# tum-vision/povar

Hardware: AMD Instinct MI355X
Metric: power-series iterations/s (solve_pOSE terms per second) (higher is better)
Workload: dtype f64

## Files before the change

povar_amd/csrc/ck_layout.hpp:

```cpp
#pragma once

#include <climits>
#include <cmath>
#include <cstring>

#include "lpl_layout.hpp"

namespace povar {

#ifndef POVAR_CK_HMAX_BUILD
#define POVAR_CK_HMAX_BUILD 16
#endif
constexpr int CK_HMAX = POVAR_CK_HMAX_BUILD;
constexpr int CK_LDS_BYTES = 160 * 1024;
constexpr int CK_FLAG_DUP = 1;
constexpr int CK_FLAG_COLD = 2;
constexpr uint32_t CK_NONE = 0xffffu;

constexpr double CK_UV_SCALE = 1e6, CK_UV_INV = 1e-6;
inline double ck_unpack_uv_host(int32_t k) {
  const double kd = (double)k;
  const double q0 = kd * CK_UV_INV;
  const double r = std::fma(-q0, CK_UV_SCALE, kd);
  return std::fma(r, CK_UV_INV, q0);
// ... 164 lines not shown
  std::vector<int> lcnt(L.tile.size() * WAVE, 0);
  lpl_parallel(grid, n_threads, [&](int w) {
    WgOut& o = out[w];
    o.bt_tiles.assign(nb, 0);
    const int t0 = L.wg_tile_off[w], t1 = L.wg_tile_off[w + 1];
    struct Ob { int key, li, src; };
    const int n_par_w = L.wg_cam_off[w + 1] - L.wg_cam_off[w];
    const int n_acc_w = std::min(n_par_w, max_acc);
    std::vector<int> acc_of_slot(n_par_w);
    std::vector<int>& acc_rank = acc_rank_of[w];
    acc_rank.resize(n_acc_w);
    if (n_acc_w == n_par_w) {
      for (int sl = 0; sl < n_par_w; ++sl) { acc_of_slot[sl] = sl; acc_rank[sl] = L.wg_cams[L.wg_cam_off[w] + sl]; }
    } else {
      std::vector<long> cnt(n_par_w, 0);
      for (int t = L.wg_tile_off[w]; t < L.wg_tile_off[w + 1]; ++t) {
        const int4 ti = L.tile[t];
        for (size_t idx = (size_t)ti.x * WAVE; idx < ((size_t)ti.x + ti.y) * WAVE; ++idx)
          if (L.cw[idx] >= 0) cnt[lpl_cw_slot(L.cw[idx])]++;
      }
      std::vector<int> by_cnt(n_par_w);
      for (int sl = 0; sl < n_par_w; ++sl) by_cnt[sl] = sl;
      std::stable_sort(by_cnt.begin(), by_cnt.end(), [&](int a, int c) { return cnt[a] > cnt[c]; });
      std::vector<char> keep(n_par_w, 0);
      for (int i = 0; i < n_acc_w; ++i) keep[by_cnt[i]] = 1;
      int a = 0;
      for (int sl = 0; sl < n_par_w; ++sl) {
        acc_of_slot[sl] = keep[sl] ? a : -1;
        if (keep[sl]) acc_rank[a++] = L.wg_cams[L.wg_cam_off[w] + sl];
        else o.capped += cnt[sl];
      }
    }
    std::vector<Ob> obs;
    std::vector<int> counts, first_of;
    struct Chunk { int key, first, len; };
    std::vector<Chunk> chunks;
    std::vector<int> assign;
    std::vector<long> cost;
    for (int b = 0; b < nb; ++b) {
      obs.clear();
      for (int t = t0 + b; t < t1; t += nb) {
        const int4 ti = L.tile[t];
        const int slot0 = ((t - t0) / nb) * WAVE;
        for (int j = 0; j < ti.y; ++j)
          for (int lane = 0; lane < WAVE; ++lane) {
            const size_t idx = ((size_t)ti.x + j) * WAVE + lane;
            const int cw = L.cw[idx];
            if (cw == -1) continue;
            Ob ob;
            if (cw >= 0) {
              const int sl = lpl_cw_slot(cw), a = acc_of_slot[sl];
              ob.key = a >= 0 ? a : n_acc_w + L.wg_cams[L.wg_cam_off[w] + sl];
            } else {
              ob.key = n_acc_w + (-2 - cw);
            }
            ob.li = slot0 + (L.seg[(size_t)t * WAVE + lane] & 255);
            ob.src = (int)idx;
            obs.push_back(ob);
            lcnt[(size_t)t * WAVE + (L.seg[(size_t)t * WAVE + lane] & 255)]++;
          }
      }
      o.obs += (int64_t)obs.size();
      std::stable_sort(obs.begin(), obs.end(), [](const Ob& a, const Ob& c) { return a.key < c.key; });
      counts.clear();
      first_of.clear();
      for (size_t i = 0; i < obs.size();) {
        size_t j = i;
        while (j < obs.size() && obs[j].key == obs[i].key) ++j;
        counts.push_back((int)(j - i));
        first_of.push_back((int)i);
        i = j;
      }
      int H = hmax, best = INT_MAX;
      for (int h = std::min(2, hmax); h <= hmax; ++h) {
        const int c = ck_schedule_cost(counts, h, n_waves, tile_overhead, nullptr);
        if (c <= best) { best = c; H = h; }
      }
      chunks.clear();
      for (size_t g = 0; g < counts.size(); ++g) {
        const int n = counts[g], k = (n + H - 1) / H, base = n / k, rem = n % k;
        int at = first_of[g];
        for (int q = 0; q < k; ++q) {
          const int len = base + (q < rem ? 1 : 0);
          chunks.push_back(Chunk{obs[at].key, at, len});
          at += len;
        }
      }
      auto rank_of = [&](int key) { return key >= n_acc_w ? key - n_acc_w : acc_rank[key]; };
      std::stable_sort(chunks.begin(), chunks.end(), [&](const Chunk& a, const Chunk& c) {
        if (a.len != c.len) return a.len > c.len;
        const int ra = rank_of(a.key), rc = rank_of(c.key);
        return ra != rc ? ra < rc : a.key < c.key;
      });
      o.chunks += (int64_t)chunks.size();
      const int n_tiles = ((int)chunks.size() + WAVE - 1) / WAVE;
      o.bt_tiles[b] = n_tiles;
      for (int tt = 0; tt < n_tiles; ++tt) {
        const int c0 = tt * WAVE, c1 = std::min((int)chunks.size(), c0 + WAVE);
        const int T = chunks[c0].len;
        int4 ti = make_int4((int)(o.uv.size() / WAVE), T, 0, (int)(o.li.size() / WAVE));
        const size_t r0 = o.uv.size(), q0 = o.li.size();
        o.uv.resize(r0 + (size_t)T * WAVE, make_double2(0, 0));
        if (shape.cold_q) o.cpos.resize(r0 + (size_t)T * WAVE, -1);
        o.src.resize(r0 + (size_t)T * WAVE, -1);
        o.li.resize(q0 + (size_t)((T + 1) / 2) * WAVE, CK_NONE | (CK_NONE << 16));
        const size_t l0 = o.lane_cam.size();
        o.lane_cam.resize(l0 + WAVE, -1);
        o.lane_acc.resize(l0 + WAVE, 0);
        o.lane_seg.resize(l0 + WAVE, 0);
        for (int lane = 0; lane < WAVE; ++lane) o.lane_seg[l0 + lane] = lane | (lane << 8);
        uint16_t occ[CK_HMAX][2][32] = {};
        uint16_t mx[CK_HMAX][2];
        for (int j = 0; j < CK_HMAX; ++j) mx[j][0] = mx[j][1] = 1;
        for (int q = c0; q < c1; ++q) {
          const int lane = q - c0, half = lane >> 5;
          const Chunk& ck = chunks[q];
          const bool cold = ck.key >= n_acc_w;
          o.lane_cam[l0 + lane] = cold ? ck.key - n_acc_w : acc_rank[ck.key];
          if (cold) {
            if (shape.cold_q) {
              o.lane_acc[l0 + lane] = -1;
              ++o.n_cold_q;
            } else {
              o.lane_acc[l0 + lane] = ~(int)o.cold_rank.size();
              o.cold_rank.push_back(ck.key - n_acc_w);
            }
            ti.z |= CK_FLAG_COLD;
          } else {
            o.lane_acc[l0 + lane] = ck.key;
            if (lane > 0 && chunks[q - 1].key == ck.key) ti.z |= CK_FLAG_DUP;
          }
          const int h = ck.len;
          assign.resize(h);
          if (place && T > 1) {
            cost.assign((size_t)T * T, 0);
            for (int a = 0; a < h; ++a) {
              const int cls = obs[ck.first + a].li & 31;
              for (int j = 0; j < T; ++j) {
                const int v = occ[j][half][cls];
                cost[(size_t)a * T + j] = 1000L * std::max(0, v + 1 - (int)mx[j][half]) + v;
              }
            }
            std::vector<int> full;
            lpl_assign(T, cost, full);
            for (int a = 0; a < h; ++a) assign[a] = full[a];
          } else {
            for (int a = 0; a < h; ++a) assign[a] = a;
          }
          for (int a = 0; a < h; ++a) {
            const Ob& ob = obs[ck.first + a];
            const int j = assign[a];
            const size_t idx = r0 + (size_t)j * WAVE + lane;
            const size_t s = (size_t)ob.src;
            o.uv[idx] = L.uv[s];
            if (shape.cold_q && cold) o.cpos[idx] = L.cpos[s];
            o.src[idx] = ob.src;
            uint32_t& word = o.li[q0 + (size_t)(j >> 1) * WAVE + lane];
            const uint32_t li3 = (uint32_t)shape.li_mul * (uint32_t)ob.li;
            word = (j & 1) ? ((word & 0xffffu) | (li3 << 16)) : ((word & 0xffff0000u) | li3);
            const uint16_t v = ++occ[j][half][ob.li & 31];
            mx[j][half] = std::max(mx[j][half], v);
          }
        }
        for (int j = 0; j < T; ++j) o.extra += (mx[j][0] - 1) + (mx[j][1] - 1);
        if (ti.z & CK_FLAG_DUP) {
          int lane = 0;
          const int nl = c1 - c0;
          while (lane < nl) {
            int e = lane;
            if (o.lane_acc[l0 + lane] >= 0)
              while (e + 1 < nl && o.lane_acc[l0 + e + 1] == o.lane_acc[l0 + lane]) ++e;
            for (int x = lane; x <= e; ++x) o.lane_seg[l0 + x] = lane | (e << 8);
            lane = e + 1;
          }
        }
        o.tile.push_back(ti);
      }
    }
  });
  K.bt_off.assign((size_t)grid * nb + 1, 0);
  std::vector<int64_t> row0_of(grid), li0_of(grid);
  std::vector<int> tile0_of(grid), cold0_of(grid);
  int n_cold_chunks = 0;
  int64_t n_cold_q = 0;
  for (int w = 0; w < grid; ++w) {
    const WgOut& o = out[w];
    row0_of[w] = K.rows;
    li0_of[w] = K.li_rows;
    tile0_of[w] = (int)K.tile.size();
    cold0_of[w] = n_cold_chunks;
    n_cold_chunks += (int)o.cold_rank.size();
    n_cold_q += o.n_cold_q;
    int t = (int)K.tile.size();
    for (int b = 0; b < nb; ++b) {
      K.bt_off[(size_t)w * nb + b] = t;
      t += o.bt_tiles[b];
      K.max_tiles_bt = std::max(K.max_tiles_bt, o.bt_tiles[b]);
    }
    for (int4 ti : o.tile) {
      ti.x += (int)K.rows;
      ti.w += (int)K.li_rows;
      K.tile.push_back(ti);
    }
    K.rows += (int64_t)(o.uv.size() / WAVE);
    K.li_rows += (int64_t)(o.li.size() / WAVE);
    K.n_chunks += o.chunks;
    K.n_obs += o.obs;
    K.n_capped_obs += o.capped;
    K.extra_lanes += o.extra;
  }
  K.bt_off[(size_t)grid * nb] = (int)K.tile.size();
  K.n_cold_chunks = n_cold_chunks + n_cold_q;
  K.cold_q = shape.cold_q;
  auto clog2 = [](int n) { int e = 0; while ((1 << e) < n) ++e; return (uint8_t)(n == 0 ? 255 : e); };
  K.lcnt_log2.resize(lcnt.size());
  for (size_t i = 0; i < lcnt.size(); ++i) K.lcnt_log2[i] = clog2(lcnt[i]);

  std::vector<int> n_rec(n_cams, 0);
  for (int w = 0; w < grid; ++w)
    for (int r0 : acc_rank_of[w]) n_rec[r0]++;
  std::vector<int> n_slot_rec(n_rec);
  for (int w = 0; w < grid; ++w)
    for (int r0 : out[w].cold_rank) n_rec[r0]++;
  std::vector<int> first(n_cams + 1, 0);
  for (int r0 = 0; r0 < n_cams; ++r0) first[r0 + 1] = first[r0] + n_rec[r0];
  K.n_part_rec = first[n_cams];
  K.part_range.assign(n_cams, make_int2(0, 0));
  for (int r0 = 0; r0 < n_cams; ++r0) K.part_range[cam_of_rank[r0]] = make_int2(first[r0], first[r0 + 1]);
  K.slot_rec.assign(L.wg_cams.size(), 0);
  {
    std::vector<int> next(first.begin(), first.end() - 1);
    for (int w = 0; w < grid; ++w)
      for (size_t a = 0; a < acc_rank_of[w].size(); ++a) K.slot_rec[(size_t)L.wg_cam_off[w] + a] = next[acc_rank_of[w][a]]++;
    std::vector<int> cold_rec((size_t)n_cold_chunks);
    for (int w = 0; w < grid; ++w)
      for (size_t i = 0; i < out[w].cold_rank.size(); ++i) cold_rec[(size_t)cold0_of[w] + i] = next[out[w].cold_rank[i]]++;
    K.uv.assign((size_t)(K.rows + CK_HMAX) * WAVE, make_double2(0, 0));
    K.src.assign((size_t)(K.rows + CK_HMAX) * WAVE, -1);
    if (shape.cold_q) K.cpos.assign((size_t)(K.rows + CK_HMAX) * WAVE, -1);
    K.li.assign((size_t)(K.li_rows + CK_HMAX) * WAVE, CK_NONE | (CK_NONE << 16));
    K.lane_cam.resize(K.tile.size() * WAVE);
    K.lane_acc.resize(K.tile.size() * WAVE);
    K.lane_seg.resize(K.tile.size() * WAVE);
    lpl_parallel(grid, n_threads, [&](int w) {
      const WgOut& o = out[w];
      std::copy(o.uv.begin(), o.uv.end(), K.uv.begin() + row0_of[w] * WAVE);
      std::copy(o.src.begin(), o.src.end(), K.src.begin() + row0_of[w] * WAVE);
      if (shape.cold_q) std::copy(o.cpos.begin(), o.cpos.end(), K.cpos.begin() + row0_of[w] * WAVE);
      std::copy(o.li.begin(), o.li.end(), K.li.begin() + li0_of[w] * WAVE);
      std::copy(o.lane_cam.begin(), o.lane_cam.end(), K.lane_cam.begin() + (size_t)tile0_of[w] * WAVE);
      std::copy(o.lane_seg.begin(), o.lane_seg.end(), K.lane_seg.begin() + (size_t)tile0_of[w] * WAVE);
      for (size_t i = 0; i < o.lane_acc.size(); ++i) {
        const int a = o.lane_acc[i];
        K.lane_acc[(size_t)tile0_of[w] * WAVE + i] = a >= 0 ? a : shape.cold_q ? -1 : ~cold_rec[(size_t)cold0_of[w] + (size_t)(~a)];
      }
    });
  }
  K.n_uv = K.uv.size();
  {
    const char* e = std::getenv("POVAR_CK_PACK");
    if (shape.need_uv && shape.slot_bytes == 48 && pack_uv && !(e && e[0] == '0')) ck_pack_uv(K, n_threads);
  }
  K.tick.assign(K.tile.size() * WAVE, 0);
  lpl_parallel(grid, n_threads, [&](int w) {
    std::vector<int> next((size_t)std::max(1, L.wg_cam_off[w + 1] - L.wg_cam_off[w]), 0);
    for (int b = 0; b < nb; ++b) {
      const int tb0 = K.bt_off[(size_t)w * nb + b], tb1 = K.bt_off[(size_t)w * nb + b + 1];
      for (int q0 = tb0; q0 < tb1; q0 += n_waves)
        for (int t = std::min(q0 + n_waves, tb1) - 1; t >= q0; --t)
          for (int lane = 0; lane < WAVE; ++lane) {
            const size_t i = (size_t)t * WAVE + lane;
            if (K.lane_cam[i] >= 0 && K.lane_acc[i] >= 0 && lane == ((K.lane_seg[i] >> 8) & 255))
              K.tick[i] = (uint16_t)next[K.lane_acc[i]]++;
          }
    }
  });
}

constexpr int CK_FIRST_PLANES = 4;
inline int ck_first_gw(int plane) { return plane == 0 ? 16 : plane == 1 ? 12 : 8; }
inline int ck_first_ng(int plane) { return plane == 3 ? 2 : 1; }
inline void ck_first_tables(const CkLayout& K, int grid, std::vector<int2>& meta, std::vector<int4>& hdr) {
  meta.assign((size_t)CK_FIRST_PLANES * grid * 16 * WAVE, make_int2(0xffff | (0xffff << 16), -1));
  hdr.assign((size_t)CK_FIRST_PLANES * grid * 16, make_int4(0, 0, 0, 0));
  const int nb = K.nb;
  auto rank16 = [&](int t, int lane) { const int r = K.lane_cam[(size_t)t * WAVE + lane]; return r < 0 ? 0xffff : (r & 0xffff); };
  for (int p = 0; p < CK_FIRST_PLANES; ++p) {
    const int gw = ck_first_gw(p), ng = ck_first_ng(p);
    for (int w = 0; w < grid; ++w)
      for (int s = 0; s < ng * gw; ++s) {
        const int b = s / gw, j = s % gw;
        if (b >= nb) continue;
        const int tb0 = K.bt_off[(size_t)w * nb + b], tb1 = K.bt_off[(size_t)w * nb + b + 1];
        const int t = tb0 + j, t2 = tb0 + gw + (gw - 1 - j);
        if (t >= tb1) continue;
        const size_t at = ((size_t)p * grid + w) * 16 + s;
        hdr[at] = K.tile[t];
        for (int lane = 0; lane < WAVE; ++lane)
          meta[at * WAVE + lane] = make_int2(rank16(t, lane) | ((t2 < tb1 ? rank16(t2, lane) : 0xffff) << 16), t);
      }
  }
}

}
```

povar_amd/csrc/povar_kernels_ck.hpp:

```cpp
#pragma once

#include "povar_kernels.hpp"

namespace povar {

constexpr int CK_ROWS = 16;

struct CkP {
  const double2* uv;
  const uint32_t* li;
  const double* w;
  const int4* tile;
  const int2* lane_meta;
  const int* bt_off;
  const int* slot_rec;
  int nb, slots;
  unsigned uv_bytes, li_bytes;
  const uint8_t* lcnt;
  const uint16_t* tick;
  int max_acc;
  int uv_packed;
  const int* cpos;
  double4* q4c;
  const int2* first_meta;
  const int4* first_hdr;
};
__device__ inline double ck_unpack_uv(unsigned k) {
  const double kd = (double)(int)k;
  const double q0 = kd * 1e-6;
  const double r = __builtin_fma(-q0, 1e6, kd);
  return __builtin_fma(r, 1e-6, q0);
}
typedef unsigned __attribute__((ext_vector_type(4))) ck_u4;
constexpr int CK_ACC_STRIDE = 13;
__host__ __device__ inline size_t ck_lds_bytes_dev(int slots, int n_acc, int ng) { return 16 + (size_t)ng * slots * 48 + (size_t)n_acc * CK_ACC_STRIDE * 8 + 64; }

__device__ inline void ck_barrier() { asm volatile("s_waitcnt lgkmcnt(0)\n\ts_barrier" ::: "memory"); }

__device__ inline void ck_group_barrier(int* cnt, int& gen, int group_waves, int lane) {
  asm volatile("s_waitcnt lgkmcnt(0)" ::: "memory");
  gen += group_waves;
  if (lane == 0) __hip_atomic_fetch_add(cnt, 1, __ATOMIC_RELAXED, __HIP_MEMORY_SCOPE_WORKGROUP);
  while (__hip_atomic_load(cnt, __ATOMIC_RELAXED, __HIP_MEMORY_SCOPE_WORKGROUP) < gen) __builtin_amdgcn_s_sleep(2);
  asm volatile("" ::: "memory");
}

__host__ __device__ inline int ck_rank(int x) { return x < 0 ? -1 : (x & 0xffff); }
__host__ __device__ inline int ck_seg(int x) { return ((x >> 16) & 63) | (((x >> 22) & 63) << 8); }

__device__ inline void ck_forward_math(const LplObs& o, const double* zz, const double* P3, double hx, double hy, double hz,
                                       double* red) {
  const double d0 = hx * zz[0] + hy * zz[1] + hz * zz[2] + zz[3];
  const double d1 = hx * zz[4] + hy * zz[5] + hz * zz[6] + zz[7];
  const double d2 = hx * zz[8] + hy * zz[9] + hz * zz[10] + zz[11];
  const double a0 = o.w * (d0 - o.cu * d2);
  const double a1 = o.w * (d1 - o.cv * d2);
  const double a2 = o.w * (o.cuv * d2 - o.cu * d0 - o.cv * d1);
  red[0] = P3[0] * a0 + P3[3] * a1 + P3[6] * a2;
  red[1] = P3[1] * a0 + P3[4] * a1 + P3[7] * a2;
  red[2] = P3[2] * a0 + P3[5] * a1 + P3[8] * a2;
}

__device__ inline double ck_huber_w(const Dp& d, const double* P3, double hx, double hy, double hz, double2 uv) {
  const double p0 = P3[0] * hx + P3[1] * hy + P3[2] * hz + P3[9];
  const double p1 = P3[3] * hx + P3[4] * hy + P3[5] * hz + P3[10];
  const double p2 = P3[6] * hx + P3[7] * hy + P3[8] * hz + P3[11];
  const double a = p0 - uv.x * p2, b = p1 - uv.y * p2, c = p0 - uv.x, e = p1 - uv.y;
  const double r2 = d.sb * d.sb * (a * a + b * b) + d.sa * d.sa * (c * c + e * e);
  const double t = d.huber;
  double y = __builtin_amdgcn_rsq(r2);
  const double hr = 0.5 * r2;
  y = y * __builtin_fma(-hr * y, y, 1.5);
  y = y * __builtin_fma(-hr * y, y, 1.5);
  return r2 < t * t ? 1.0 : t * y;
}

__device__ inline void ck_obs_forward(const Dp& d, double2 uv, double w, const double* zz, const double* P3, double hx, double hy,
                                      double hz, double* lu, int S, uint32_t s) {
  LplObs o;
  o.set(d, uv, w);
  double red[3];
  ck_forward_math(o, zz, P3, hx, hy, hz, red);
  __hip_atomic_fetch_add(lu + s, red[0], __ATOMIC_RELAXED, __HIP_MEMORY_SCOPE_WORKGROUP);
  __hip_atomic_fetch_add(lu + s + 1, red[1], __ATOMIC_RELAXED, __HIP_MEMORY_SCOPE_WORKGROUP);
  __hip_atomic_fetch_add(lu + s + 2, red[2], __ATOMIC_RELAXED, __HIP_MEMORY_SCOPE_WORKGROUP);
}
__device__ inline void ck_obs_backward(const Dp& d, double2 uv, double w, const double* P3, double hx, double hy, double hz,
                                       const double* g, double* y) {
  LplObs o;
  o.set(d, uv, w);
  double q[3];
  lpl_backward(o, P3, g, q);
#pragma unroll
  for (int m = 0; m < 3; ++m) {
    y[4 * m] += hx * q[m];
    y[4 * m + 1] += hy * q[m];
    y[4 * m + 2] += hz * q[m];
    y[4 * m + 3] += q[m];
  }
}

struct CkRows {
  __amdgpu_buffer_rsrc_t uv, li, w;
};
__device__ inline CkRows ck_rows(const CkP& k) {
  CkRows R;
  R.uv = __builtin_amdgcn_make_buffer_rsrc(const_cast<double2*>(k.uv), 0, k.uv_bytes, 0x00020000);
  R.li = __builtin_amdgcn_make_buffer_rsrc(const_cast<uint32_t*>(k.li), 0, k.li_bytes, 0x00020000);
  R.w = __builtin_amdgcn_make_buffer_rsrc(const_cast<double*>(k.w), 0, k.w ? (k.uv_packed ? k.uv_bytes : k.uv_bytes / 2) : 0, 0x00020000);
  return R;
}
template <int D, bool ROBUST, bool PK = false>
struct CkStream {
  double2 uv[D];
  unsigned pk[D][2];
  uint32_t w[D];
  __device__ inline void clear() {
#pragma unroll
    for (int i = 0; i < D; ++i) {
      uv[i] = make_double2(0, 0);
      pk[i][0] = pk[i][1] = 0;
      w[i] = 0xffffffffu;
    }
  }
  __device__ inline double2 get(int i) const { return PK ? make_double2(ck_unpack_uv(pk[i][0]), ck_unpack_uv(pk[i][1])) : uv[i]; }
  __device__ inline void load(const CkRows& R, int row0, int li0, int j, int h, int lane, int i) {
    j = j < 0 ? 0 : (j >= h ? h - 1 : j);
    const unsigned ul = (unsigned)lane;
    const unsigned ro = (unsigned)(row0 + j) * (unsigned)(WAVE * 16), lo = (unsigned)(li0 + (j >> 1)) * (unsigned)(WAVE * 4);
    if (PK) {
      typedef unsigned __attribute__((ext_vector_type(2))) u2;
      const u2 a = __builtin_amdgcn_raw_buffer_load_b64(R.uv, ul * 8u, ro >> 1, 0);
      pk[i][0] = a.x;
      pk[i][1] = a.y;
    } else {
      typedef unsigned __attribute__((ext_vector_type(4))) u4;
      const u4 a = __builtin_amdgcn_raw_buffer_load_b128(R.uv, ul * 16u, ro, 0);
      uv[i] = make_double2(__longlong_as_double(((long long)a.y << 32) | a.x), __longlong_as_double(((long long)a.w << 32) | a.z));
    }
    w[i] = __builtin_amdgcn_raw_buffer_load_b32(R.li, ul * 4u, lo, 0);
  }
  template <int DIR>
  __device__ inline void start(const CkRows& R, int row0, int li0, int h, int lane) {
#pragma unroll
    for (int i = 0; i < D; ++i) load(R, row0, li0, DIR > 0 ? i : h - 1 - i, h, lane, i);
  }
};
template <int D, bool ROBUST, bool PK>
__device__ inline void ck_forward_step(const Dp& d, const CkRows& k, CkStream<D, ROBUST, PK>& st, int row0, int li0, int h, int lane,
                                       const double* zz, const double* P3, const double* lh, double* lu, int S, int j, int i) {
  const double2 uv = st.get(i);
  const uint32_t s = (st.w[i] >> (16 * (j & 1))) & 0xffffu;
  st.load(k, row0, li0, j + D, h, lane, i);
  if (s != 0xffffu) {
    const double hx = lh[s], hy = lh[s + 1], hz = lh[s + 2];
    const double rw = ROBUST ? ck_huber_w(d, P3, hx, hy, hz, uv) : 1.0;
    ck_obs_forward(d, uv, rw, zz, P3, hx, hy, hz, lu, S, s);
  }
}
template <int D, bool ROBUST, bool PK>
__device__ inline void ck_forward_rows(const Dp& d, const CkRows& k, CkStream<D, ROBUST, PK>& st, int row0, int li0, int h, int lane,
                                       const double* zz, const double* P3, const double* lh, double* lu, int S) {
  int n0 = 0;
#pragma nounroll
  for (; n0 + D <= h; n0 += D) {
#pragma unroll
    for (int i = 0; i < D; ++i) ck_forward_step<D, ROBUST, PK>(d, k, st, row0, li0, h, lane, zz, P3, lh, lu, S, n0 + i, i);
  }
#pragma unroll
  for (int i = 0; i < D - 1; ++i)
    if (n0 + i < h) ck_forward_step<D, ROBUST, PK>(d, k, st, row0, li0, h, lane, zz, P3, lh, lu, S, n0 + i, i);
}
template <int D, bool ROBUST, bool PK>
__device__ inline void ck_backward_step(const Dp& d, const CkRows& k, CkStream<D, ROBUST, PK>& st, int row0, int li0, int h, int lane,
                                        const double* P3, const double* lh, const double* lg, int S, double* y, int j, int i) {
  const double2 uv = st.get(i);
  const uint32_t s = (st.w[i] >> (16 * (j & 1))) & 0xffffu;
  st.load(k, row0, li0, j - D, h, lane, i);
  if (s != 0xffffu) {
    const double hx = lh[s], hy = lh[s + 1], hz = lh[s + 2];
    const double rw = ROBUST ? ck_huber_w(d, P3, hx, hy, hz, uv) : 1.0;
    const double g[3] = {lg[s], lg[s + 1], lg[s + 2]};
    ck_obs_backward(d, uv, rw, P3, hx, hy, hz, g, y);
  }
}
template <int D, bool ROBUST, bool PK>
__device__ inline void ck_backward_rows(const Dp& d, const CkRows& k, CkStream<D, ROBUST, PK>& st, int row0, int li0, int h, int lane,
                                        const double* P3, const double* lh, const double* lg, int S, double* y) {
  int n0 = 0;
#pragma nounroll
  for (; n0 + D <= h; n0 += D) {
#pragma unroll
    for (int i = 0; i < D; ++i) ck_backward_step<D, ROBUST, PK>(d, k, st, row0, li0, h, lane, P3, lh, lg, S, y, h - 1 - (n0 + i), i);
  }
#pragma unroll
  for (int i = 0; i < D - 1; ++i)
    if (n0 + i < h) ck_backward_step<D, ROBUST, PK>(d, k, st, row0, li0, h, lane, P3, lh, lg, S, y, h - 1 - (n0 + i), i);
}

template <bool ROBUST, bool PK>
__device__ inline void ck_backward_rows_cold(const Dp& d, const CkP& k, const CkRows& R, int row0, int li0, int h, int lane,
                                             const double* P3, const double* lh, const double* lg, bool cold_lane, double* y) {
  for (int j = h - 1; j >= 0; --j) {
    CkStream<2, ROBUST, PK> one;
    one.load(R, row0, li0, j, h, lane, 0);
    const int cp = cold_lane ? k.cpos[(size_t)(row0 + j) * WAVE + lane] : -1;
    const double2 uv = one.get(0);
    const uint32_t s = (one.w[0] >> (16 * (j & 1))) & 0xffffu;
    if (s != 0xffffu) {
      const double hx = lh[s], hy = lh[s + 1], hz = lh[s + 2];
      const double rw = ROBUST ? ck_huber_w(d, P3, hx, hy, hz, uv) : 1.0;
      const double g[3] = {lg[s], lg[s + 1], lg[s + 2]};
      LplObs o;
      o.set(d, uv, rw);
      double q[3];
      lpl_backward(o, P3, g, q);
      if (cp >= 0) {
        k.q4c[cp] = make_double4(q[0], q[1], q[2], 0.0);
      } else {
#pragma unroll
        for (int m = 0; m < 3; ++m) {
          y[4 * m] += hx * q[m];
          y[4 * m + 1] += hy * q[m];
          y[4 * m + 2] += hz * q[m];
          y[4 * m + 3] += q[m];
        }
      }
    }
  }
}

__device__ inline void ck_load_z(const Dp& d, int rank, double* zz) {
  const double2* r = reinterpret_cast<const double2*>(d.hot_rec + (size_t)rank * HOT_REC_STRIDE);
#pragma unroll
  for (int j = 0; j < 6; ++j) {
    const double2 v = r[j];
    zz[2 * j] = v.x;
    zz[2 * j + 1] = v.y;
  }
}
__device__ inline __amdgpu_buffer_rsrc_t ck_zimg_rsrc(const Dp& d) {
  return __builtin_amdgcn_make_buffer_rsrc(d.zimg, 0, (unsigned)d.n_cams * 96u, 0x00020000);
}
__device__ inline void ck_load_z_img(const Dp& d, int rank, double* zz) {
  const __amdgpu_buffer_rsrc_t ZR = ck_zimg_rsrc(d);
#pragma unroll
  for (int j = 0; j < 6; ++j) {
    const ck_u4 a = __builtin_amdgcn_raw_buffer_load_b128(ZR, (unsigned)rank * 96u + 16u * j, 0, 0);
    zz[2 * j] = __hiloint2double((int)a.y, (int)a.x);
    zz[2 * j + 1] = __hiloint2double((int)a.w, (int)a.z);
  }
}
__device__ inline void ck_load_p3(const Dp& d, int rank, double* P3) {
  const double2* r = reinterpret_cast<const double2*>(d.hot_rec + (size_t)rank * HOT_REC_STRIDE) + 6;
#pragma unroll
  for (int j = 0; j < 4; ++j) {
    const double2 v = r[j];
    P3[2 * j] = v.x;
    P3[2 * j + 1] = v.y;
  }
  P3[8] = d.hot_rec[(size_t)rank * HOT_REC_STRIDE + 20];
}
template <bool ROBUST>
__device__ inline void ck_load_p(const Dp& d, int rank, double* P3) {
  ck_load_p3(d, rank, P3);
  if (ROBUST) {
    const double* r = d.hot_rec + (size_t)rank * HOT_REC_STRIDE;
    P3[9] = r[21];
    const double2 v = reinterpret_cast<const double2*>(r)[11];
    P3[10] = v.x;
    P3[11] = v.y;
  }
}

#ifndef POVAR_CK_PART_AUX
#define POVAR_CK_PART_AUX 0
#endif
__device__ inline __amdgpu_buffer_rsrc_t ck_part_rsrc(double* part_out) {
  return __builtin_amdgcn_make_buffer_rsrc(part_out, 0, 0x7ffffff0, 0x00020000);
}
__device__ inline void ck_store_part(__amdgpu_buffer_rsrc_t pr, unsigned byte_off, double a, double b) {
  ck_u4 g;
  g.x = (unsigned)__double2loint(a); g.y = (unsigned)__double2hiint(a); g.z = (unsigned)__double2loint(b); g.w = (unsigned)__double2hiint(b);
  __builtin_amdgcn_raw_buffer_store_b128(g, pr, byte_off, 0, POVAR_CK_PART_AUX);
}
__device__ inline void ck_flush_tile(double (&y)[12], int flags, int lane, int rank, int acc_slot, int seg, double* acc, int n_acc,
                                     double* part_ptr) {
  if (flags & 1) seg_scan_steps<12>(y, lane, seg & 255, 4);
  if (rank >= 0) {
    if (acc_slot >= 0) {
      if (lane == ((seg >> 8) & 255)) {
#pragma unroll
        for (int m = 0; m < 12; ++m)
          __hip_atomic_fetch_add(acc + acc_slot * CK_ACC_STRIDE + m, y[m], __ATOMIC_RELAXED, __HIP_MEMORY_SCOPE_WORKGROUP);
      }
    } else if (part_ptr) {
      const __amdgpu_buffer_rsrc_t part_out = ck_part_rsrc(part_ptr);
      const unsigned o = (unsigned)(~acc_slot) * 96u;
#pragma unroll
      for (int m = 0; m < 6; ++m) ck_store_part(part_out, o + 16u * m, y[2 * m], y[2 * m + 1]);
    }
  }
}

template <int NW, int SD, bool DB, int NG, bool ROBUST, bool PK>
__global__ __launch_bounds__(NW * 64) void e0_ck(Dp d, CkP k, double* part_out) {
  const int done = d.flags[1];
  extern __shared__ double ck_lds[];
  constexpr int GW = NW / NG;
  const CkRows R = ck_rows(k);
  const int S = k.slots;
  const int lane0 = threadIdx.x & 63;
  const int wave_all = __builtin_amdgcn_readfirstlane((int)(threadIdx.x >> 6));
  const int grp = NG > 1 ? wave_all / GW : 0;
  const int wave = NG > 1 ? wave_all % GW : wave_all;
  int* gbase = reinterpret_cast<int*>(ck_lds);
  double* lh = ck_lds + 2 + (size_t)grp * 6 * S;
  double* lu = lh + 3 * S;
  double* acc = ck_lds + 2 + (size_t)NG * 6 * S;
  int* gcnt = gbase + grp;
  int ggen = 0;
  const V2& v = d.v2;
  const int cam0 = v.wg_cam_off[blockIdx.x];
  const int n_acc = v.wg_cam_off[blockIdx.x + 1] - cam0;
  const int t0 = __builtin_amdgcn_readfirstlane(v.wg_tile_off[blockIdx.x]);
  const int t1 = __builtin_amdgcn_readfirstlane(v.wg_tile_off[blockIdx.x + 1]);
  typedef const int __attribute__((address_space(4))) * cint_p;
  const cint_p tiles = (cint_p)(uintptr_t)k.tile;
  const cint_p bt = (cint_p)(uintptr_t)k.bt_off;
  if (done) return;
  auto group_barrier = [&]() {
    if (NG > 1) ck_group_barrier(gcnt, ggen, GW, lane0);
    else ck_barrier();
  };
  const int wave_t = (wave & ~3) | (((wave >> 2) & 1) ? 3 - (wave & 3) : (wave & 3));
  auto tile_of = [&](int tb0, int q) { return tb0 + q * GW + ((q & 1) ? GW - 1 - wave_t : wave_t); };
  constexpr int HM = 32 / NW > 0 ? 32 / NW : 1;
  double hn[HM][3];
  auto request_h = [&](int b, int lane) {
#pragma unroll
    for (int q = 0; q < HM; ++q) {
      hn[q][0] = hn[q][1] = hn[q][2] = 0;
      const int m = wave + q * GW;
      if (b < k.nb && t0 + b + k.nb * m < t1) {
        const double* rp = v.lmrec + ((size_t)(t0 + b + k.nb * m) * 9) * WAVE + lane;
        hn[q][0] = rp[0]; hn[q][1] = rp[WAVE]; hn[q][2] = rp[2 * WAVE];
      }
    }
  };
  int* lbt = reinterpret_cast<int*>(acc + (size_t)k.max_acc * CK_ACC_STRIDE);
  const bool bt_lds = k.nb + 1 <= 16;
  auto bt_of = [&](int i, bool first) {
    return (bt_lds && !first) ? __builtin_amdgcn_readfirstlane(lbt[i]) : bt[blockIdx.x * k.nb + i];
  };
  constexpr bool EARLY = !ROBUST && SD == 2;
  int tb0_next = 0, tb1_next = 0, rank_next = 0, rank_next2 = 0;
  ck_u4 hdr_next = {0, 0, 0, 0};
  auto request_first_meta = [&](int b, int lane, bool ranks) {
    tb0_next = tb1_next = 0;
    if (b < k.nb) {
      tb0_next = bt_of(b, b == grp);
      tb1_next = bt_of(b + 1, b == grp);
    }
    if (!ranks) return;
    rank_next = rank_next2 = 0;
    hdr_next = ck_u4{0, 0, 0, 0};
    if (b < k.nb) {
      const int tf = tile_of(tb0_next, 0), tf2 = tile_of(tb0_next, 1);
      if (tf < tb1_next && !EARLY) rank_next = ck_rank(k.lane_meta[(size_t)tf * WAVE + lane].x);
      if (tf < tb1_next && EARLY) {
        const __amdgpu_buffer_rsrc_t TR = __builtin_amdgcn_make_buffer_rsrc(const_cast<int4*>(k.tile), 0, 0x7ffffff0, 0x00020000);
        hdr_next = __builtin_amdgcn_raw_buffer_load_b128(TR, 0u, (unsigned)tf * 16u, 0);
        rank_next = ck_rank(k.lane_meta[(size_t)tf * WAVE + lane].x);
        if (tf2 < tb1_next) rank_next2 = ck_rank(k.lane_meta[(size_t)tf2 * WAVE + lane].x);
      }
    }
  };
  double zz[12] = {0, 0, 0, 0, 0, 0, 0, 0, 0, 0, 0, 0}, P3[12] = {0, 0, 0, 0, 0, 0, 0, 0, 0, 0, 0, 0};
  CkStream<SD, ROBUST, PK> st;
  st.clear();
  int row0 = 0, h = 0, fl = 0, li0 = 0;
  auto request_first_tile = [&](int lane, bool have) {
    const int tf = tile_of(tb0_next, 0);
    const int rk = rank_next < 0 ? 0 : rank_next;
    if (have && EARLY) {
      row0 = __builtin_amdgcn_readfirstlane((int)hdr_next.x);
      h = __builtin_amdgcn_readfirstlane((int)hdr_next.y);
      fl = __builtin_amdgcn_readfirstlane((int)hdr_next.z);
      li0 = __builtin_amdgcn_readfirstlane((int)hdr_next.w);
      ck_load_z_img(d, rk, zz);
      ck_load_p<ROBUST>(d, rk, P3);
      st.template start<1>(R, row0, li0, h, lane);
    } else if (have) {
      const int tf2 = tile_of(tb0_next, 1);
      row0 = tiles[4 * tf]; h = tiles[4 * tf + 1]; fl = tiles[4 * tf + 2]; li0 = tiles[4 * tf + 3];
      if (tf2 < tb1_next) rank_next2 = ck_rank(k.lane_meta[(size_t)tf2 * WAVE + lane].x);
      ck_load_p<ROBUST>(d, rk, P3);
      st.template start<1>(R, row0, li0, h, lane);
      ck_load_z_img(d, rk, zz);
    } else {
#pragma unroll
      for (int e = 0; e < 12; ++e) zz[e] = P3[e] = 0;
      st.clear();
      row0 = h = fl = li0 = 0;
    }
  };
  int bt_first = 0;
  if (bt_lds && (int)threadIdx.x <= k.nb) bt_first = k.bt_off[blockIdx.x * k.nb + threadIdx.x];
  if (EARLY) {
    static_assert(!EARLY || (NG == 1 && (GW == 16 || GW == 12 || GW == 8)) || (NG == 2 && GW == 8), "shape without a first-request table");
    constexpr int PLANE = NG > 1 ? 3 : GW == 16 ? 0 : GW == 12 ? 1 : 2;
    const unsigned fs = (PLANE * gridDim.x + blockIdx.x) * 16u + (unsigned)(grp * GW + wave_t);
    const int2 fm = k.first_meta[(size_t)fs * WAVE + lane0];
    const __amdgpu_buffer_rsrc_t HR = __builtin_amdgcn_make_buffer_rsrc(const_cast<int4*>(k.first_hdr), 0, 0x7ffffff0, 0x00020000);
    hdr_next = __builtin_amdgcn_raw_buffer_load_b128(HR, 0u, fs * 16u, 0);
    request_h(grp, lane0);
    const int r1 = fm.x & 0xffff, r2 = (fm.x >> 16) & 0xffff;
    rank_next = r1 == 0xffff ? -1 : r1;
    rank_next2 = r2 == 0xffff ? -1 : r2;
    request_first_tile(lane0, __builtin_amdgcn_readfirstlane(fm.y) >= 0);
    request_first_meta(grp, lane0, false);
  } else {
    request_first_meta(grp, lane0, true);
    request_h(grp, lane0);
  }
  for (int i = threadIdx.x; i < n_acc * CK_ACC_STRIDE; i += NW * 64) acc[i] = 0;
  if (NG > 1 && threadIdx.x < NG) gbase[threadIdx.x] = 0;
  if (bt_lds && (int)threadIdx.x <= k.nb) lbt[threadIdx.x] = bt_first;
  if (NG > 1) ck_barrier();
  for (int b = grp; b < k.nb; b += NG) {
    int lane = lane0;
    asm volatile("" : "+v"(lane));
    const int tb0 = tb0_next, tb1 = tb1_next;
    int q_t = 0;
    int t = tile_of(tb0, 0);
    int rank = rank_next;
    int tn = tile_of(tb0, 1);
    if (!EARLY) request_first_tile(lane, t < tb1);
    int rank_n = rank_next2, rank_nn = 0;
    double zn[12] = {0, 0, 0, 0, 0, 0, 0, 0, 0, 0, 0, 0}, Pn[12] = {0, 0, 0, 0, 0, 0, 0, 0, 0, 0, 0, 0};
    CkStream<SD, ROBUST, PK> stn;
    stn.clear();
    int row0n = 0, hnx = 0, fln = 0, li0n = 0;
#pragma unroll
    for (int q = 0; q < HM; ++q) {
      const int m = wave + q * GW;
      if (t0 + b + k.nb * m < t1) {
        const int s = m * WAVE + lane;
        lh[3 * s] = hn[q][0];
        lh[3 * s + 1] = hn[q][1];
        lh[3 * s + 2] = hn[q][2];
        lu[3 * s] = 0;
        lu[3 * s + 1] = 0;
        lu[3 * s + 2] = 0;
      }
    }
    for (int m = wave + HM * GW; t0 + b + k.nb * m < t1; m += GW) {
      const double* rp = v.lmrec + ((size_t)(t0 + b + k.nb * m) * 9) * WAVE + lane;
      const int s = m * WAVE + lane;
      lh[3 * s] = rp[0];
      lh[3 * s + 1] = rp[WAVE];
      lh[3 * s + 2] = rp[2 * WAVE];
      lu[3 * s] = 0;
      lu[3 * s + 1] = 0;
      lu[3 * s + 2] = 0;
    }
    auto request_next_fwd = [&]() {
      if (DB && tn < tb1) {
        const int tnn = tile_of(tb0, q_t + 2);
        row0n = tiles[4 * tn]; hnx = tiles[4 * tn + 1]; fln = tiles[4 * tn + 2]; li0n = tiles[4 * tn + 3];
        if (tnn < tb1) rank_nn = ck_rank(k.lane_meta[(size_t)tnn * WAVE + lane].x);
        const int rk = rank_n < 0 ? 0 : rank_n;
        ck_load_z_img(d, rk, zn);
        ck_load_p<ROBUST>(d, rk, Pn);
        stn.template start<1>(R, row0n, li0n, hnx, lane);
      }
    };
    request_next_fwd();
    group_barrier();
#pragma unroll
    for (int e = 0; e < 12; ++e) asm volatile("" : "+v"(zz[e]));
    while (t < tb1) {
      ck_forward_rows<SD, ROBUST, PK>(d, R, st, row0, li0, h, lane, zz, P3, lh, lu, S);
      if (tn >= tb1) break;
      t = tn;
      ++q_t;
      rank = rank_n;
      tn = tile_of(tb0, q_t + 1);
      if (DB) {
#pragma unroll
        for (int e = 0; e < 12; ++e) zz[e] = zn[e];
#pragma unroll
        for (int e = 0; e < (ROBUST ? 12 : 9); ++e) P3[e] = Pn[e];
        st = stn;
        row0 = row0n; h = hnx; fl = fln; li0 = li0n;
        rank_n = rank_nn;
        request_next_fwd();
      } else {
        row0 = tiles[4 * t]; h = tiles[4 * t + 1]; fl = tiles[4 * t + 2]; li0 = tiles[4 * t + 3];
        if (tn < tb1) rank_n = ck_rank(k.lane_meta[(size_t)tn * WAVE + lane].x);
        const int rk = rank < 0 ? 0 : rank;
        ck_load_z_img(d, rk, zz);
        ck_load_p<ROBUST>(d, rk, P3);
        st.template start<1>(R, row0, li0, h, lane);
      }
    }
    asm volatile("" : "+v"(lane));
    int acc_slot = 0, seg = 0;
    int tp = q_t > 0 ? tile_of(tb0, q_t - 1) : tb1;
    int rank_p = 0, acc_p = 0, seg_p = 0, rank_pp = 0, acc_pp = 0, seg_pp = 0;
    double G[HM][6];
#pragma unroll
    for (int q = 0; q < HM; ++q) {
#pragma unroll
      for (int e = 0; e < 6; ++e) G[q][e] = 0;
      const int m = wave + q * GW;
      if (t0 + b + k.nb * m < t1) {
        const double* rp = v.lmrec + ((size_t)(t0 + b + k.nb * m) * 9 + 3) * WAVE + lane;
#pragma unroll
        for (int e = 0; e < 6; ++e) G[q][e] = rp[e * WAVE];
      }
    }
    if (t < tb1) {
      const int2 me = k.lane_meta[(size_t)t * WAVE + lane];
      seg = ck_seg(me.x);
      acc_slot = me.y;
      if (tp < tb1) {
        const int2 mp = k.lane_meta[(size_t)tp * WAVE + lane];
        rank_p = ck_rank(mp.x);
        seg_p = ck_seg(mp.x);
        acc_p = mp.y;
      }
      st.template start<-1>(R, row0, li0, h, lane);
    }
    group_barrier();
    request_first_meta(b + NG, lane, true);
    request_h(b + NG, lane);
#pragma unroll
    for (int q = 0; q < HM; ++q) {
      const int m = wave + q * GW;
      if (t0 + b + k.nb * m < t1) {
        const int s = m * WAVE + lane;
        const double u0 = lu[3 * s], u1 = lu[3 * s + 1], u2 = lu[3 * s + 2];
        lu[3 * s] = G[q][0] * u0 + G[q][1] * u1 + G[q][2] * u2;
        lu[3 * s + 1] = G[q][1] * u0 + G[q][3] * u1 + G[q][4] * u2;
        lu[3 * s + 2] = G[q][2] * u0 + G[q][4] * u1 + G[q][5] * u2;
      }
    }
    for (int m = wave + HM * GW; t0 + b + k.nb * m < t1; m += GW) {
      const double* rp = v.lmrec + ((size_t)(t0 + b + k.nb * m) * 9 + 3) * WAVE + lane;
      const double g0 = rp[0], g1 = rp[WAVE], g2 = rp[2 * WAVE], g3 = rp[3 * WAVE], g4 = rp[4 * WAVE], g5 = rp[5 * WAVE];
      const int s = m * WAVE + lane;
      const double u0 = lu[3 * s], u1 = lu[3 * s + 1], u2 = lu[3 * s + 2];
      lu[3 * s] = g0 * u0 + g1 * u1 + g2 * u2;
      lu[3 * s + 1] = g1 * u0 + g3 * u1 + g4 * u2;
      lu[3 * s + 2] = g2 * u0 + g4 * u1 + g5 * u2;
    }
    auto request_next_bwd = [&]() {
      if (DB && tp < tb1) {
        const int tpp = q_t > 1 ? tile_of(tb0, q_t - 2) : tb1;
        row0n = tiles[4 * tp]; hnx = tiles[4 * tp + 1]; fln = tiles[4 * tp + 2]; li0n = tiles[4 * tp + 3];
        if (tpp < tb1) {
          const int2 mp = k.lane_meta[(size_t)tpp * WAVE + lane];
          rank_pp = ck_rank(mp.x);
          seg_pp = ck_seg(mp.x);
          acc_pp = mp.y;
        }
        ck_load_p<ROBUST>(d, rank_p < 0 ? 0 : rank_p, Pn);
        stn.template start<-1>(R, row0n, li0n, hnx, lane);
      }
    };
    request_next_bwd();
    group_barrier();
    while (t < tb1) {
      double y[12];
#pragma unroll
      for (int m = 0; m < 12; ++m) y[m] = 0;
      const bool cold_q = !ROBUST && k.cpos != nullptr && (fl & 2) != 0;
      if (cold_q) ck_backward_rows_cold<ROBUST, PK>(d, k, R, row0, li0, h, lane, P3, lh, lu, rank >= 0 && acc_slot < 0, y);
      else ck_backward_rows<SD, ROBUST, PK>(d, R, st, row0, li0, h, lane, P3, lh, lu, S, y);
      ck_flush_tile(y, fl, lane, rank, acc_slot, seg, acc, n_acc, cold_q ? nullptr : part_out);
      if (tp >= tb1) break;
      t = tp;
      --q_t;
      rank = rank_p; acc_slot = acc_p; seg = seg_p;
      tp = q_t > 0 ? tile_of(tb0, q_t - 1) : tb1;
      if (DB) {
#pragma unroll
        for (int e = 0; e < (ROBUST ? 12 : 9); ++e) P3[e] = Pn[e];
        st = stn;
        row0 = row0n; h = hnx; fl = fln; li0 = li0n;
        rank_p = rank_pp; acc_p = acc_pp; seg_p = seg_pp;
        request_next_bwd();
      } else {
        row0 = tiles[4 * t]; h = tiles[4 * t + 1]; fl = tiles[4 * t + 2]; li0 = tiles[4 * t + 3];
        if (tp < tb1) {
          const int2 mp = k.lane_meta[(size_t)tp * WAVE + lane];
          rank_p = ck_rank(mp.x);
          seg_p = ck_seg(mp.x);
          acc_p = mp.y;
        }
        ck_load_p<ROBUST>(d, rank < 0 ? 0 : rank, P3);
        st.template start<-1>(R, row0, li0, h, lane);
      }
    }
    if (EARLY) request_first_tile(lane, tile_of(tb0_next, 0) < tb1_next);
    group_barrier();
  }
  if (NG > 1) ck_barrier();
  const __amdgpu_buffer_rsrc_t PR = ck_part_rsrc(part_out);
  for (int i = threadIdx.x; i < n_acc * 6; i += NW * 64) {
    const int r = i / 6, m = 2 * (i % 6);
    const int rec = k.slot_rec[cam0 + r];
    ck_store_part(PR, (unsigned)rec * 96u + 16u * (unsigned)(i % 6), acc[r * CK_ACC_STRIDE + m], acc[r * CK_ACC_STRIDE + m + 1]);
  }
  if (d.p2p_epoch && blockIdx.x == 0 && threadIdx.x == 0) *d.p2p_epoch += 1;
}

POVAR_KERNEL __launch_bounds__(256) void ck_gather_w(const int* src, const double* w_lpl, double* w_ck, int64_t n) {
  const int64_t i = (int64_t)blockIdx.x * 256 + threadIdx.x;
  if (i >= n) return;
  const int s = src[i];
  w_ck[i] = s >= 0 ? w_lpl[s] : 0.0;
}

}
```

Baseline: 19390.

## Defer lane-meta decoding and add optional ticket-based barrier scheduling

For the early, single-group, 16-wave shape, the per-block lane-meta decode is deferred: raw metadata is loaded before the barrier and decoded after it, and the next-block meta and h prefetch is moved after the G·u update so it overlaps differently. A ticket mechanism is added, built on an atomic counter in LDS. It can redistribute the G-matrix loads across the first-arriving waves and let late waves use a hardware barrier instead of spinning. The ticket paths are disabled by default (POVAR_CK_TICKET=0), but the deferral path is always on for matching shapes. This changes register live ranges and barrier timing in exchange for hiding metadata load latency.

```diff
diff --git a/povar_amd/csrc/ck_layout.hpp b/povar_amd/csrc/ck_layout.hpp
--- a/povar_amd/csrc/ck_layout.hpp
+++ b/povar_amd/csrc/ck_layout.hpp
@@ -490,4 +490,10 @@
   }
 }
 
-}
+constexpr int ck_ticket_w(int gw) { return gw - gw / 4; }
+__host__ __device__ inline int ck_ticket_slot_tile(int ticket, int w, int q, int n) {
+  const int m = ticket + q * w;
+  return ticket < w && m < n ? m : -1;
+}
+
+}
diff --git a/povar_amd/csrc/povar_kernels_ck.hpp b/povar_amd/csrc/povar_kernels_ck.hpp
--- a/povar_amd/csrc/povar_kernels_ck.hpp
+++ b/povar_amd/csrc/povar_kernels_ck.hpp
@@ -1,6 +1,7 @@
 #pragma once
 
 #include "povar_kernels.hpp"
+#include "ck_layout.hpp"
 
 namespace povar {
 
@@ -44,6 +45,20 @@
   while (__hip_atomic_load(cnt, __ATOMIC_RELAXED, __HIP_MEMORY_SCOPE_WORKGROUP) < gen) __builtin_amdgcn_s_sleep(2);
   asm volatile("" ::: "memory");
 }
+
+__device__ inline int ck_ticket(int* cnt, int& gen, int waves, int lane) {
+  int t = 0;
+  if (lane == 0) t = __hip_atomic_fetch_add(cnt, 1, __ATOMIC_RELAXED, __HIP_MEMORY_SCOPE_WORKGROUP);
+  t = __builtin_amdgcn_readfirstlane(t) - gen;
+  gen += waves;
+  return t;
+}
+#ifndef POVAR_CK_TICKET
+#define POVAR_CK_TICKET 0
+#endif
+#ifndef POVAR_CK_TICKET_LATE
+#define POVAR_CK_TICKET_LATE 2
+#endif
 
 __host__ __device__ inline int ck_rank(int x) { return x < 0 ? -1 : (x & 0xffff); }
 __host__ __device__ inline int ck_seg(int x) { return ((x >> 16) & 63) | (((x >> 22) & 63) << 8); }
@@ -354,6 +369,16 @@
     return (bt_lds && !first) ? __builtin_amdgcn_readfirstlane(lbt[i]) : bt[blockIdx.x * k.nb + i];
   };
   constexpr bool EARLY = !ROBUST && SD == 2;
+  constexpr bool DEFER = EARLY && NG == 1 && !DB && NW == 16;
+  constexpr bool TICKET = EARLY && NG == 1 && !DB && NW == 16;
+  constexpr bool TK_END = TICKET && (POVAR_CK_TICKET & 1) != 0, TK_B2 = TICKET && (POVAR_CK_TICKET & 2) != 0;
+#ifdef POVAR_CK_TICKET_W
+  constexpr int TK_LATE = POVAR_CK_TICKET_LATE, TK_W = POVAR_CK_TICKET_W;
+#else
+  constexpr int TK_LATE = POVAR_CK_TICKET_LATE, TK_W = ck_ticket_w(GW);
+#endif
+  constexpr int HMG = TK_B2 ? (HM * GW + TK_W - 1) / TK_W : HM;
+  int tk_gen = 0;
   int tb0_next = 0, tb1_next = 0, rank_next = 0, rank_next2 = 0;
   ck_u4 hdr_next = {0, 0, 0, 0};
   auto request_first_meta = [&](int b, int lane, bool ranks) {
@@ -371,8 +396,13 @@
       if (tf < tb1_next && EARLY) {
         const __amdgpu_buffer_rsrc_t TR = __builtin_amdgcn_make_buffer_rsrc(const_cast<int4*>(k.tile), 0, 0x7ffffff0, 0x00020000);
         hdr_next = __builtin_amdgcn_raw_buffer_load_b128(TR, 0u, (unsigned)tf * 16u, 0);
-        rank_next = ck_rank(k.lane_meta[(size_t)tf * WAVE + lane].x);
-        if (tf2 < tb1_next) rank_next2 = ck_rank(k.lane_meta[(size_t)tf2 * WAVE + lane].x);
+        if (DEFER) {
+          rank_next = k.lane_meta[(size_t)tf * WAVE + lane].x;
+          if (tf2 < tb1_next) rank_next2 = k.lane_meta[(size_t)tf2 * WAVE + lane].x;
+        } else {
+          rank_next = ck_rank(k.lane_meta[(size_t)tf * WAVE + lane].x);
+          if (tf2 < tb1_next) rank_next2 = ck_rank(k.lane_meta[(size_t)tf2 * WAVE + lane].x);
+        }
       }
     }
   };
@@ -382,7 +412,7 @@
   int row0 = 0, h = 0, fl = 0, li0 = 0;
   auto request_first_tile = [&](int lane, bool have) {
     const int tf = tile_of(tb0_next, 0);
-    const int rk = rank_next < 0 ? 0 : rank_next;
+    const int rk = DEFER ? (ck_rank(rank_next) < 0 ? 0 : ck_rank(rank_next)) : rank_next < 0 ? 0 : rank_next;
     if (have && EARLY) {
       row0 = __builtin_amdgcn_readfirstlane((int)hdr_next.x);
       h = __builtin_amdgcn_readfirstlane((int)hdr_next.y);
@@ -426,6 +456,8 @@
   }
   for (int i = threadIdx.x; i < n_acc * CK_ACC_STRIDE; i += NW * 64) acc[i] = 0;
   if (NG > 1 && threadIdx.x < NG) gbase[threadIdx.x] = 0;
+  if (TICKET && threadIdx.x == 0) gbase[0] = 0;
+  const int n_st0 = TK_B2 ? (t1 - t0) / k.nb : 0, n_st_rem = TK_B2 ? (t1 - t0) % k.nb : 0;
   if (bt_lds && (int)threadIdx.x <= k.nb) lbt[threadIdx.x] = bt_first;
   if (NG > 1) ck_barrier();
   for (int b = grp; b < k.nb; b += NG) {
@@ -434,10 +466,10 @@
     const int tb0 = tb0_next, tb1 = tb1_next;
     int q_t = 0;
     int t = tile_of(tb0, 0);
-    int rank = rank_next;
+    int rank = DEFER ? ck_rank(rank_next) : rank_next;
     int tn = tile_of(tb0, 1);
     if (!EARLY) request_first_tile(lane, t < tb1);
-    int rank_n = rank_next2, rank_nn = 0;
+    int rank_n = DEFER ? ck_rank(rank_next2) : rank_next2, rank_nn = 0;
     double zn[12] = {0, 0, 0, 0, 0, 0, 0, 0, 0, 0, 0, 0}, Pn[12] = {0, 0, 0, 0, 0, 0, 0, 0, 0, 0, 0, 0};
     CkStream<SD, ROBUST, PK> stn;
     stn.clear();
@@ -509,52 +541,104 @@
     int acc_slot = 0, seg = 0;
     int tp = q_t > 0 ? tile_of(tb0, q_t - 1) : tb1;
     int rank_p = 0, acc_p = 0, seg_p = 0, rank_pp = 0, acc_pp = 0, seg_pp = 0;
-    double G[HM][6];
-#pragma unroll
-    for (int q = 0; q < HM; ++q) {
-#pragma unroll
-      for (int e = 0; e < 6; ++e) G[q][e] = 0;
-      const int m = wave + q * GW;
-      if (t0 + b + k.nb * m < t1) {
+    const int tk = TK_B2 ? ck_ticket(gbase, tk_gen, GW, lane0) : 0;
+    const bool late = TK_B2 && tk >= GW - TK_LATE;
+    const int n_st = n_st0 + (b < n_st_rem ? 1 : 0);
+    double G[HMG][6];
+    if constexpr (!TK_B2) {
+#pragma unroll
+      for (int q = 0; q < HM; ++q) {
+#pragma unroll
+        for (int e = 0; e < 6; ++e) G[q][e] = 0;
+        const int m = wave + q * GW;
+        if (t0 + b + k.nb * m < t1) {
+          const double* rp = v.lmrec + ((size_t)(t0 + b + k.nb * m) * 9 + 3) * WAVE + lane;
+#pragma unroll
+          for (int e = 0; e < 6; ++e) G[q][e] = rp[e * WAVE];
+        }
+      }
+    }
+    if (late) ck_barrier();
+    int2 me_b = make_int2(0, 0), mp_b = make_int2(0, 0);
+    if constexpr (!DEFER) {
+      if (t < tb1) {
+        const int2 me = k.lane_meta[(size_t)t * WAVE + lane];
+        seg = ck_seg(me.x);
+        acc_slot = me.y;
+        if (tp < tb1) {
+          const int2 mp = k.lane_meta[(size_t)tp * WAVE + lane];
+          rank_p = ck_rank(mp.x);
+          seg_p = ck_seg(mp.x);
+          acc_p = mp.y;
+        }
+        st.template start<-1>(R, row0, li0, h, lane);
+      }
+    } else if (t < tb1) {
+      me_b = k.lane_meta[(size_t)t * WAVE + lane];
+      if (tp < tb1) mp_b = k.lane_meta[(size_t)tp * WAVE + lane];
+      st.template start<-1>(R, row0, li0, h, lane);
+    }
+    if constexpr (TK_B2) {
+#pragma unroll
+      for (int q = 0; q < HMG; ++q) {
+#pragma unroll
+        for (int e = 0; e < 6; ++e) G[q][e] = 0;
+        const int m = ck_ticket_slot_tile(tk, TK_W, q, n_st);
+        if (m >= 0) {
+          const double* rp = v.lmrec + ((size_t)(t0 + b + k.nb * m) * 9 + 3) * WAVE + lane;
+#pragma unroll
+          for (int e = 0; e < 6; ++e) G[q][e] = rp[e * WAVE];
+        }
+      }
+    }
+    if (!late) group_barrier();
+    if (!DEFER) {
+      request_first_meta(b + NG, lane, true);
+      request_h(b + NG, lane);
+    }
+    if constexpr (!TK_B2) {
+#pragma unroll
+      for (int q = 0; q < HM; ++q) {
+        const int m = wave + q * GW;
+        if (t0 + b + k.nb * m < t1) {
+          const int s = m * WAVE + lane;
+          const double u0 = lu[3 * s], u1 = lu[3 * s + 1], u2 = lu[3 * s + 2];
+          lu[3 * s] = G[q][0] * u0 + G[q][1] * u1 + G[q][2] * u2;
+          lu[3 * s + 1] = G[q][1] * u0 + G[q][3] * u1 + G[q][4] * u2;
+          lu[3 * s + 2] = G[q][2] * u0 + G[q][4] * u1 + G[q][5] * u2;
+        }
+      }
+      for (int m = wave + HM * GW; t0 + b + k.nb * m < t1; m += GW) {
         const double* rp = v.lmrec + ((size_t)(t0 + b + k.nb * m) * 9 + 3) * WAVE + lane;
-#pragma unroll
-        for (int e = 0; e < 6; ++e) G[q][e] = rp[e * WAVE];
-      }
-    }
-    if (t < tb1) {
-      const int2 me = k.lane_meta[(size_t)t * WAVE + lane];
-      seg = ck_seg(me.x);
-      acc_slot = me.y;
-      if (tp < tb1) {
-        const int2 mp = k.lane_meta[(size_t)tp * WAVE + lane];
-        rank_p = ck_rank(mp.x);
-        seg_p = ck_seg(mp.x);
-        acc_p = mp.y;
-      }
-      st.template start<-1>(R, row0, li0, h, lane);
-    }
-    group_barrier();
-    request_first_meta(b + NG, lane, true);
-    request_h(b + NG, lane);
-#pragma unroll
-    for (int q = 0; q < HM; ++q) {
-      const int m = wave + q * GW;
-      if (t0 + b + k.nb * m < t1) {
+        const double g0 = rp[0], g1 = rp[WAVE], g2 = rp[2 * WAVE], g3 = rp[3 * WAVE], g4 = rp[4 * WAVE], g5 = rp[5 * WAVE];
         const int s = m * WAVE + lane;
         const double u0 = lu[3 * s], u1 = lu[3 * s + 1], u2 = lu[3 * s + 2];
-        lu[3 * s] = G[q][0] * u0 + G[q][1] * u1 + G[q][2] * u2;
-        lu[3 * s + 1] = G[q][1] * u0 + G[q][3] * u1 + G[q][4] * u2;
-        lu[3 * s + 2] = G[q][2] * u0 + G[q][4] * u1 + G[q][5] * u2;
-      }
-    }
-    for (int m = wave + HM * GW; t0 + b + k.nb * m < t1; m += GW) {
-      const double* rp = v.lmrec + ((size_t)(t0 + b + k.nb * m) * 9 + 3) * WAVE + lane;
-      const double g0 = rp[0], g1 = rp[WAVE], g2 = rp[2 * WAVE], g3 = rp[3 * WAVE], g4 = rp[4 * WAVE], g5 = rp[5 * WAVE];
-      const int s = m * WAVE + lane;
-      const double u0 = lu[3 * s], u1 = lu[3 * s + 1], u2 = lu[3 * s + 2];
-      lu[3 * s] = g0 * u0 + g1 * u1 + g2 * u2;
-      lu[3 * s + 1] = g1 * u0 + g3 * u1 + g4 * u2;
-      lu[3 * s + 2] = g2 * u0 + g4 * u1 + g5 * u2;
+        lu[3 * s] = g0 * u0 + g1 * u1 + g2 * u2;
+        lu[3 * s + 1] = g1 * u0 + g3 * u1 + g4 * u2;
+        lu[3 * s + 2] = g2 * u0 + g4 * u1 + g5 * u2;
+      }
+    } else {
+      auto g_u = [&](int m, double g0, double g1, double g2, double g3, double g4, double g5) {
+        const int s = m * WAVE + lane;
+        const double u0 = lu[3 * s], u1 = lu[3 * s + 1], u2 = lu[3 * s + 2];
+        lu[3 * s] = g0 * u0 + g1 * u1 + g2 * u2;
+        lu[3 * s + 1] = g1 * u0 + g3 * u1 + g4 * u2;
+        lu[3 * s + 2] = g2 * u0 + g4 * u1 + g5 * u2;
+      };
+#pragma unroll
+      for (int q = 0; q < HMG; ++q) {
+        const int m = ck_ticket_slot_tile(tk, TK_W, q, n_st);
+        if (m >= 0) g_u(m, G[q][0], G[q][1], G[q][2], G[q][3], G[q][4], G[q][5]);
+      }
+      for (int q = HMG; ck_ticket_slot_tile(tk, TK_W, q, n_st) >= 0; ++q) {
+        const int m = ck_ticket_slot_tile(tk, TK_W, q, n_st);
+        const double* rp = v.lmrec + ((size_t)(t0 + b + k.nb * m) * 9 + 3) * WAVE + lane;
+        g_u(m, rp[0], rp[WAVE], rp[2 * WAVE], rp[3 * WAVE], rp[4 * WAVE], rp[5 * WAVE]);
+      }
+    }
+    if (DEFER) {
+      request_first_meta(b + NG, lane, true);
+      request_h(b + NG, lane);
     }
     auto request_next_bwd = [&]() {
       if (DB && tp < tb1) {
@@ -572,6 +656,13 @@
     };
     request_next_bwd();
     group_barrier();
+    if (DEFER) {
+      seg = ck_seg(me_b.x);
+      acc_slot = me_b.y;
+      rank_p = ck_rank(mp_b.x);
+      seg_p = ck_seg(mp_b.x);
+      acc_p = mp_b.y;
+    }
     while (t < tb1) {
       double y[12];
 #pragma unroll
@@ -604,8 +695,11 @@
         st.template start<-1>(R, row0, li0, h, lane);
       }
     }
+    const int tk_e = TK_END && b + NG < k.nb ? ck_ticket(gbase, tk_gen, GW, lane0) : 0;
+    const bool late_e = TK_END && tk_e >= GW - TK_LATE;
+    if (late_e) ck_barrier();
     if (EARLY) request_first_tile(lane, tile_of(tb0_next, 0) < tb1_next);
-    group_barrier();
+    if (!late_e) group_barrier();
   }
   if (NG > 1) ck_barrier();
   const __amdgpu_buffer_rsrc_t PR = ck_part_rsrc(part_out);
```

Result: faster. 19660, median of 6 (+1.4%).
